# sahaRatul/sela

Hardware: AMD Instinct MI355X
Metric: Msamples/s encode+decode, 16-bit stereo 44.1kHz, 1/2/4/8 GPU; bit-exact vs CPU (higher is better)
Workload: dtype f64+int64

## Files before the change

### include/sela_hip_debug.h

```cpp
#ifndef SELA_HIP_DEBUG_H_
#define SELA_HIP_DEBUG_H_

#include <stddef.h>
#include <stdint.h>

#ifdef __cplusplus
extern "C" {
#endif

void sela_hip_debug_phase_buffer(uint64_t* d_cycles);
void sela_hip_debug_force_plain_fir(int enable);
void sela_hip_debug_mean_workers(int self_blocks);
void sela_hip_debug_encode_teams(int lanes);
int sela_hip_debug_encode_kernel(uint32_t n_frames, uint32_t channels);
void sela_hip_debug_encode_fused(int enable);
void sela_hip_debug_priorities(uint32_t team_quarters);
void sela_hip_debug_priorities_adaptive(void);
int sela_hip_debug_launches_alone(void);
void sela_hip_debug_keep_both_candidates(int on);
void sela_hip_debug_stage_wait(int naps);
int sela_hip_debug_reissued_feeds(void);
void sela_hip_debug_decode_recurrence(int form);
int sela_hip_debug_contexts_created(void);
void sela_hip_debug_coalesced(int kind, long long* batches, long long* retried);
size_t sela_hip_debug_verify_lds_bytes(uint32_t channels);
size_t sela_hip_debug_levels_lds_bytes(uint32_t channels);
size_t sela_hip_debug_digest_lds_bytes(uint32_t channels);
long long sela_hip_debug_verify_i32_fallback_frames(const void* d_workspace, uint32_t max_frames, uint32_t channels, uint32_t stride);
long long sela_hip_debug_verify_pcm_fallback_frames(const void* d_workspace, uint32_t max_frames, uint32_t channels, uint32_t stride);
long long sela_hip_debug_levels_i32_fallback_frames(const void* d_workspace, uint32_t max_frames, uint32_t channels, uint32_t stride);

void sela_hip_debug_encode_hashes(int on);
int sela_hip_debug_block_forms(const void* d_workspace, uint32_t n_frames, uint32_t channels, uint32_t* counts_out, uint8_t* forms_out);
void sela_hip_debug_encode_split(int mode);
int sela_hip_debug_launches_split(void);
void sela_hip_debug_standard_first(int mode);
int sela_hip_debug_standard_chunks(void);
long long sela_hip_debug_segment_subframes(void);
void sela_hip_debug_generic_wrap_taps(int on);
size_t sela_hip_debug_window_lds_bytes(uint32_t channels);
uint64_t sela_hip_debug_windows_staged_bytes(void);
enum {
    SELA_HIP_WORKSPACE_ENCODE = 0, SELA_HIP_WORKSPACE_DECODE, SELA_HIP_WORKSPACE_INDEX, SELA_HIP_WORKSPACE_DECODE_I32, SELA_HIP_WORKSPACE_DECODE_N,
    SELA_HIP_WORKSPACE_VERIFY, SELA_HIP_WORKSPACE_VERIFY_I32, SELA_HIP_WORKSPACE_ENCODE_I32, SELA_HIP_WORKSPACE_ENCODE_PAIRED, SELA_HIP_WORKSPACE_WINDOWS,
    SELA_HIP_WORKSPACE_WINDOWS_WHOLE, SELA_HIP_WORKSPACE_ENCODE_WHOLE, SELA_HIP_WORKSPACE_ENCODE_SPLIT, SELA_HIP_WORKSPACE_DECODE_WHOLE, SELA_HIP_WORKSPACE_WINDOWS_I32,
    SELA_HIP_WORKSPACE_WINDOWS_I32_WHOLE, SELA_HIP_WORKSPACE_ENCODE_WHOLE_PCM
};
int sela_hip_debug_workspace_pieces(int call, uint64_t a, uint32_t b, uint32_t c, uint64_t* offset_bytes_pairs, int capacity);
void sela_hip_debug_pcm_chunk_frames(uint32_t frames);

#ifdef __cplusplus
}
#endif
#endif
```

### sela_amd/capi.py

```python
from __future__ import annotations

import ctypes as C
import os

HERE = os.path.dirname(os.path.abspath(__file__))
LIB_PATH = os.path.join(HERE, "libsela_hip.so")

OK = 0
ERRORS = {-1: "ENODEV", -2: "EINVAL", -3: "ENOMEM", -4: "ECAPACITY", -5: "EFORMAT", -6: "ERANGE"}
SAMPLES_PER_FRAME = 2048

FLAG_Q_RANGE, FLAG_COEF_OVERFLOW, FLAG_RICE_RANGE, FLAG_RICE_OVERRUN, FLAG_WORDS_CAP, FLAG_BAD_FRAME, FLAG_INTERNAL, FLAG_SHORT_BLOCK = 1, 2, 4, 8, 16, 32, 64, 128
FLAG_STRIDE = 256

EXPORTS = [
    "sela_hip_init", "sela_hip_shutdown", "sela_hip_thread_release", "sela_hip_last_error", "sela_hip_device_count",
    "sela_hip_signals_per_frame", "sela_hip_encode_workspace_bytes", "sela_hip_decode_workspace_bytes",
    "sela_hip_encode_bound_bytes", "sela_hip_encode_device", "sela_hip_decode_device",
    "sela_hip_encode", "sela_hip_decode", "sela_hip_index_frames",
    "sela_hip_enable_kernel_timing", "sela_hip_kernel_times",
    "sela_hip_lpc_encode", "sela_hip_lpc_decode", "sela_hip_rice_encode", "sela_hip_rice_decode",
    "sela_hip_host_alloc", "sela_hip_host_free", "sela_hip_decode_max_channels",
    "sela_hip_encode_begin", "sela_hip_encode_feed", "sela_hip_encode_end",
    "sela_hip_decode_begin", "sela_hip_decode_feed", "sela_hip_decode_end",
# ... 6 lines not shown
    "sela_hip_verify_workspace_bytes", "sela_hip_verify_device", "sela_hip_verify_payload_device", "sela_hip_verify",
    "sela_hip_verify_i32_workspace_bytes", "sela_hip_verify_i32_device", "sela_hip_verify_payload_i32_device", "sela_hip_verify_i32",
    "sela_hip_encode_device_opt", "sela_hip_encode_n_device_opt", "sela_hip_encode_i32_device_opt", "sela_hip_encode_opt", "sela_hip_encode_i32_opt",
    "sela_hip_encode_ragged_i32_opt", "sela_hip_encode_begin_opt",
    "sela_hip_decode_windows_workspace_bytes", "sela_hip_decode_windows_device", "sela_hip_decode_windows",
    "sela_hip_decode_windows_whole_workspace_bytes", "sela_hip_decode_windows_whole_device", "sela_hip_decode_windows_whole",
    "sela_hip_decode_windows_i32_workspace_bytes", "sela_hip_decode_windows_i32_device", "sela_hip_decode_windows_i32",
    "sela_hip_decode_windows_i32_whole_workspace_bytes", "sela_hip_decode_windows_i32_whole_device", "sela_hip_decode_windows_i32_whole",
    "sela_hip_encode_whole_pcm_bound_bytes", "sela_hip_encode_whole_pcm_workspace_bytes", "sela_hip_encode_whole_pcm_device", "sela_hip_encode_whole_pcm",
    "sela_hip_paired_signals_per_frame", "sela_hip_encode_paired_workspace_bytes", "sela_hip_encode_paired_i32_device", "sela_hip_encode_paired_n_device",
    "sela_hip_encode_paired_i32", "sela_hip_encode_paired",
    "sela_hip_whole_frames", "sela_hip_whole_frame", "sela_hip_encode_whole_bound_bytes", "sela_hip_encode_whole_workspace_bytes",
    "sela_hip_encode_whole_device", "sela_hip_encode_whole",
    "sela_hip_decode_whole_workspace_bytes", "sela_hip_decode_whole_device", "sela_hip_decode_whole_payload_device", "sela_hip_decode_whole_status_error",
    "sela_hip_decode_whole",
    "sela_hip_pcm_unpack_device", "sela_hip_pcm_pack_device", "sela_hip_encode_pcm_workspace_bytes", "sela_hip_encode_pcm_bound_bytes",
    "sela_hip_encode_pcm_device", "sela_hip_decode_pcm_workspace_bytes", "sela_hip_decode_pcm_device", "sela_hip_decode_pcm_status_error",
    "sela_hip_encode_pcm", "sela_hip_decode_pcm",
    "sela_hip_verify_pcm_workspace_bytes", "sela_hip_verify_pcm_device", "sela_hip_verify_payload_pcm_device", "sela_hip_verify_pcm",
    "sela_hip_levels_workspace_bytes", "sela_hip_levels_device", "sela_hip_levels_payload_device", "sela_hip_levels",
    "sela_hip_levels_i32_workspace_bytes", "sela_hip_levels_i32_device", "sela_hip_levels_payload_i32_device", "sela_hip_levels_samples_i32_workspace_bytes",
    "sela_hip_levels_samples_i32_device", "sela_hip_levels_i32",
    "sela_hip_digest_workspace_bytes", "sela_hip_digest_device", "sela_hip_digest_payload_device", "sela_hip_digest", "sela_hip_crc32_combine",
    "sela_hip_crc32_workspace_bytes", "sela_hip_crc32_device",
]
WINDOW_I16_INTERLEAVED, WINDOW_F32_PLANAR = 0, 1
WINDOW_I32_PLANAR, WINDOW_PCM24_INTERLEAVED, WINDOW_PCM32_INTERLEAVED = 2, 3, 4
ENCODE_LOSSLESS = 1



DEBUG_EXPORTS = [
    "sela_hip_debug_phase_buffer", "sela_hip_debug_force_plain_fir", "sela_hip_debug_mean_workers", "sela_hip_debug_encode_teams", "sela_hip_debug_encode_kernel", "sela_hip_debug_encode_fused", "sela_hip_debug_priorities", "sela_hip_debug_priorities_adaptive", "sela_hip_debug_launches_alone", "sela_hip_debug_block_forms", "sela_hip_debug_encode_hashes", "sela_hip_debug_standard_first", "sela_hip_debug_standard_chunks", "sela_hip_debug_segment_subframes", "sela_hip_debug_generic_wrap_taps", "sela_hip_debug_encode_split", "sela_hip_debug_launches_split", "sela_hip_debug_keep_both_candidates", "sela_hip_debug_stage_wait",
    "sela_hip_debug_reissued_feeds", "sela_hip_debug_contexts_created", "sela_hip_debug_decode_recurrence", "sela_hip_debug_coalesced", "sela_hip_debug_verify_lds_bytes",
    "sela_hip_debug_verify_i32_fallback_frames", "sela_hip_debug_window_lds_bytes", "sela_hip_debug_windows_staged_bytes",
    "sela_hip_debug_workspace_pieces", "sela_hip_debug_pcm_chunk_frames", "sela_hip_debug_verify_pcm_fallback_frames",
    "sela_hip_debug_levels_lds_bytes", "sela_hip_debug_levels_i32_fallback_frames", "sela_hip_debug_digest_lds_bytes",
]
WORKSPACE_CALLS = ("encode", "decode", "index", "decode_i32", "decode_n", "verify", "verify_i32", "encode_i32", "encode_paired", "windows", "windows_whole",
                   "encode_whole", "encode_split", "decode_whole", "windows_i32", "windows_i32_whole", "encode_whole_pcm")


class Trace(C.Structure):
    _fields_ = [
        ("mean", C.c_double), ("ac", C.c_double * 101), ("k", C.c_double * 100), ("a", C.c_int64 * 101),
        ("q", C.c_int32 * 100), ("order", C.c_int32), ("coef_k", C.c_uint32), ("coef_words", C.c_uint32),
        ("res_k", C.c_uint32), ("res_words", C.c_uint32), ("flags", C.c_uint32),
    ]


class SelaHipError(RuntimeError):
    def __init__(self, code: int, message: str):
        super().__init__(f"libsela_hip: {ERRORS.get(code, code)}: {message}")
        self.code = code


_LIB = None


def lib() -> C.CDLL:
    global _LIB
    if _LIB is not None:
        return _LIB
    if not os.path.exists(LIB_PATH):
        raise ImportError(
            f"{LIB_PATH} is missing: build it with `python -c 'import __graft_entry__ as g; g.build()'` "
            "(hipcc --offload-arch=gfx950).  The SELA MI355X path has no CPU fallback.")
# ... 240 lines not shown
    L.sela_hip_debug_encode_fused.restype = None
    L.sela_hip_debug_priorities.argtypes = [C.c_uint32]
    L.sela_hip_debug_priorities.restype = None
    L.sela_hip_debug_priorities_adaptive.argtypes = []
    L.sela_hip_debug_priorities_adaptive.restype = None
    L.sela_hip_debug_launches_alone.argtypes = []
    L.sela_hip_debug_launches_alone.restype = C.c_int
    L.sela_hip_debug_encode_hashes.argtypes = [C.c_int]
    L.sela_hip_debug_encode_hashes.restype = None
    L.sela_hip_debug_standard_first.argtypes = [C.c_int]
    L.sela_hip_debug_standard_first.restype = None
    L.sela_hip_debug_standard_chunks.argtypes = []
    L.sela_hip_debug_standard_chunks.restype = C.c_int
    L.sela_hip_debug_segment_subframes.argtypes = []
    L.sela_hip_debug_segment_subframes.restype = C.c_longlong
    L.sela_hip_debug_generic_wrap_taps.argtypes = [C.c_int]
    L.sela_hip_debug_generic_wrap_taps.restype = None
    L.sela_hip_debug_encode_split.argtypes = [C.c_int]
    L.sela_hip_debug_encode_split.restype = None
    L.sela_hip_debug_launches_split.argtypes = []
    L.sela_hip_debug_launches_split.restype = C.c_int
    L.sela_hip_debug_block_forms.argtypes = [C.c_void_p, C.c_uint32, C.c_uint32, C.c_void_p, C.c_void_p]
    L.sela_hip_debug_block_forms.restype = C.c_int
    L.sela_hip_debug_keep_both_candidates.argtypes = [C.c_int]
    L.sela_hip_debug_keep_both_candidates.restype = None
    L.sela_hip_debug_encode_kernel.argtypes = [C.c_uint32, C.c_uint32]
    L.sela_hip_debug_encode_kernel.restype = C.c_int
    L.sela_hip_debug_stage_wait.argtypes = [C.c_int]
    L.sela_hip_debug_stage_wait.restype = None
    L.sela_hip_debug_reissued_feeds.argtypes = []
    L.sela_hip_debug_reissued_feeds.restype = C.c_int
    L.sela_hip_debug_decode_recurrence.argtypes = [C.c_int]
    L.sela_hip_debug_decode_recurrence.restype = None
    L.sela_hip_debug_contexts_created.argtypes = []
    L.sela_hip_debug_contexts_created.restype = C.c_int
    L.sela_hip_debug_coalesced.argtypes = [C.c_int, C.POINTER(C.c_longlong), C.POINTER(C.c_longlong)]
    L.sela_hip_debug_coalesced.restype = None
    L.sela_hip_debug_verify_lds_bytes.argtypes = [u32]
    L.sela_hip_debug_verify_lds_bytes.restype = sz
    L.sela_hip_debug_verify_i32_fallback_frames.argtypes = [vp, u32, u32, u32]
    L.sela_hip_debug_verify_pcm_fallback_frames.argtypes = [vp, u32, u32, u32]
    L.sela_hip_debug_verify_pcm_fallback_frames.restype = C.c_longlong
    L.sela_hip_debug_verify_i32_fallback_frames.restype = C.c_longlong
    L.sela_hip_debug_window_lds_bytes.argtypes = [u32]
    L.sela_hip_debug_window_lds_bytes.restype = sz
    L.sela_hip_debug_windows_staged_bytes.argtypes = []
    L.sela_hip_debug_windows_staged_bytes.restype = C.c_uint64
    L.sela_hip_debug_workspace_pieces.argtypes = [C.c_int, u64, u32, u32, u64p, C.c_int]
    L.sela_hip_debug_workspace_pieces.restype = C.c_int
    L.sela_hip_host_alloc.argtypes = [sz]
    L.sela_hip_host_alloc.restype = C.c_void_p
    L.sela_hip_host_free.argtypes = [C.c_void_p]
    L.sela_hip_host_free.restype = None
    L.sela_hip_decode_max_channels.argtypes = []
    L.sela_hip_decode_max_channels.restype = u32
    L.sela_hip_encode_begin.argtypes = [C.POINTER(C.c_void_p), u32, u32, vp, sz, vp]
    L.sela_hip_encode_feed.argtypes = [vp, vp, u32, C.POINTER(C.c_uint32), C.POINTER(C.c_uint64)]
    L.sela_hip_encode_end.argtypes = [vp, C.POINTER(C.c_uint32), C.POINTER(C.c_uint64)]
    L.sela_hip_decode_begin.argtypes = [C.POINTER(C.c_void_p), u32, u32, vp]
    L.sela_hip_decode_feed.argtypes = [vp, vp, vp, u32, C.POINTER(C.c_uint32)]
    L.sela_hip_decode_end.argtypes = [vp, C.POINTER(C.c_uint32)]
    for name in ("sela_hip_encode_begin", "sela_hip_encode_feed", "sela_hip_encode_end", "sela_hip_decode_begin",
                 "sela_hip_decode_feed", "sela_hip_decode_end"):
        getattr(L, name).restype = C.c_int
    _LIB = L
    return L
# ... 22 lines not shown
```

### sela_amd/csrc/sela_capi.hip

```cpp
#include <hip/hip_runtime.h>

#include <algorithm>
#include <atomic>

#include <chrono>
#include <condition_variable>
#include <deque>
#include <thread>
#include <cstdio>
#include <cstdlib>
#include <cstring>
#include <map>
#include <mutex>
#include <string>
#include <vector>

#include "sela_coalescer.h"
#include "sela_crc32.h"
#include "sela_decode_whole_plan.h"
#include "sela_host.h"
#include "sela_lease.h"
#include "sela_pcm.h"

namespace {
// ... 1147 lines not shown
    if (e == hipSuccess && blocks) {
        const size_t head = first ? (size_t)first * n_sig : blocks;
        if (!first)
            e = hipMemcpy(meta.data(), sela::encode_block_records(d_workspace, n_frames, channels), blocks * sizeof(sela::BlockMeta), hipMemcpyDeviceToHost);
        else {
            sela::Carve c(d_workspace);
            const SplitWs halves = carve_encode_split(c, first, n_frames - first, channels);
            e = hipMemcpy(meta.data(), sela::encode_block_records(halves.first, first, channels), head * sizeof(sela::BlockMeta), hipMemcpyDeviceToHost);
            if (e == hipSuccess)
                e = hipMemcpy(meta.data() + head, sela::encode_block_records(halves.second, n_frames - first, channels), (blocks - head) * sizeof(sela::BlockMeta),
                    hipMemcpyDeviceToHost);
        }
    }
    if (e != hipSuccess)
        return fail_hip(e, "block forms");
    for (size_t b = 0; b < blocks; b++) {
        const uint32_t form = (meta[b].flags & sela::kBlockFormPlain) ? 2 : ((meta[b].flags & sela::kBlockFormTwoPass) ? 1 : 0);
        counts_out[form]++;
        if (forms_out)
            forms_out[b] = (uint8_t)form;
    }
    return SELA_HIP_OK;
}
void sela_hip_debug_keep_both_candidates(int on) { sela::set_keep_both_candidates(on); }
void sela_hip_debug_encode_split(int mode) { g_encode_split.store(mode < 0 || mode > 999 ? 0 : mode, std::memory_order_relaxed); }
int sela_hip_debug_launches_split(void) { return g_launches_split.load(std::memory_order_relaxed); }
void sela_hip_debug_encode_hashes(int on) { sela::set_encode_hashes(on); }
int sela_hip_debug_encode_kernel(uint32_t n_frames, uint32_t channels) { return sela::encode_team_lanes(n_frames, channels, g_team_lanes); }

void sela_hip_debug_stage_wait(int naps) { g_stage_wait_naps = naps; }

int sela_hip_debug_reissued_feeds(void) { return g_reissued_feeds; }
void sela_hip_debug_decode_recurrence(int form) { g_recurrence_form = form < 0 ? -1 : (form != 0); }
int sela_hip_debug_contexts_created(void) { return g_contexts_created.load(std::memory_order_relaxed); }

void sela_hip_enable_kernel_timing(int enable) { g_timing.enabled = enable != 0; }

int sela_hip_kernel_times(float* ms_out, int capacity)
{
    const int n = g_timing.recorded < capacity ? g_timing.recorded : capacity;
    for (int i = 0; i < n; i++) {
        if (hipEventSynchronize(g_timing.ev[i + 1]) != hipSuccess || hipEventElapsedTime(&ms_out[i], g_timing.ev[i], g_timing.ev[i + 1]) != hipSuccess)
            return 0;
    }
    return n;
}

uint32_t sela_hip_signals_per_frame(uint32_t channels) { return channels == 2 ? 3u : channels; }

size_t sela_hip_encode_workspace_bytes(uint32_t n_frames, uint32_t channels)
{
    const size_t whole = sela::encode_workspace_bytes(n_frames, channels);
    return sela::encode_split_frames(n_frames, channels, 500) ? whole + sela::encode_workspace_bytes(0, channels) + 65536 : whole;
}

size_t sela_hip_decode_workspace_bytes(uint32_t n_frames, uint32_t channels) { return sela::decode_workspace_bytes(n_frames, channels); }

uint32_t sela_hip_decode_max_channels(void) { return sela::decode_max_channels(); }

size_t sela_hip_encode_bound_bytes(uint32_t n_frames, uint32_t channels)
{
    return (size_t)n_frames * sela_frame_bytes(channels, channels * (uint32_t)sela::kSlotWords);
}

namespace {
int encode_device_call(const int16_t* d_pcm, uint32_t n_frames, uint32_t channels, uint8_t* d_frames, size_t frames_cap,
// ... 2129 lines not shown
```

### sela_amd/csrc/sela_decode.hip

```cpp
#include <atomic>

#include "sela_host.h"

#include "sela_synth.h"

namespace sela {

#include "sela_decode_core.inc"

template <bool kProf>
__global__ __launch_bounds__(kDecMaxWaves * 64) __attribute__((amdgpu_waves_per_eu(7, 8))) void k_decode_frames(const uint8_t* __restrict__ frames,
    const uint64_t* __restrict__ frame_offsets, uint32_t n_frames, uint32_t channels, int16_t* __restrict__ pcm_out,
    uint32_t* __restrict__ status, int32_t* __restrict__ ws_residues, uint64_t* __restrict__ phase_cycles,
    uint8_t* __restrict__ frame_flags ,
    uint32_t vec_shift_from ,
    uint32_t synth_priorities ,
    const uint32_t* __restrict__ n_frames_found )
{
    long long stamp[10];
    for (int i = 0; i < 10; i++)
        stamp[i] = 0;
    uint32_t prof_sub = kNoSubframe;
    if (kProf)
        stamp[0] = clock64();
    extern __shared__ __attribute__((aligned(16))) unsigned char dyn[];
    const int n_waves = blockDim.x / 64;
    const int wave = __builtin_amdgcn_readfirstlane((int)(threadIdx.x / 64)), lane = threadIdx.x % 64;
    const DecFrameLds l = carve_frame_lds(dyn, channels, n_waves);

    const uint32_t f = blockIdx.x;
    if (f >= n_frames || (n_frames_found && f >= *n_frames_found))
        return;
    const bool vec_shift = f >= vec_shift_from;
    const uint8_t* const fb = frames + frame_offsets[f];
    const uint64_t fbytes = frame_offsets[f + 1] - frame_offsets[f];
    uint32_t flags = 0;
    SubHeader hd;
    bool ok;
    const bool fast = frame_prologue(l, fb, fbytes, channels, n_waves, wave, lane, hd, ok);
    if (kProf)
        stamp[1] = clock64();

    for (uint32_t c = wave; c < channels; c += n_waves) {
        if (c != (uint32_t)wave) {
            hd = walk_headers(fb, fbytes, c);
            ok = block_header_ok(hd, channels);
        }
        if (!ok) {
            flags |= SELA_HIP_FLAG_BAD_FRAME;
            continue;
        }
        if (kProf)
            prof_sub = c;
        decode_subframe<kProf>(fb, fbytes, hd, fast, l.sub + c, l.scratch0 + wave, ws_residues, (size_t)f * channels + c, vec_shift, synth_priorities, lane, flags, stamp);
        if (lane == 0)
            l.sub_info[hd.channel] = sub_info_word(hd.type, hd.parent, c);
    }
    __syncthreads();

    if (channels == 2) {
        const StereoPass sp = stereo_pass(l.sub, l.sub_info);
        uint4* out = reinterpret_cast<uint4*>(pcm_out + (size_t)f * kBlock * 2);
        for (uint32_t i4 = threadIdx.x; i4 < (uint32_t)kBlock / 4; i4 += blockDim.x)
            out[i4] = stereo_words(sp, i4);
    } else {
        for (uint32_t i = threadIdx.x; i < (uint32_t)kBlock; i += blockDim.x)
            for (uint32_t c = 0; c < channels; c++)
                pcm_out[((size_t)f * kBlock + i) * channels + c] = (int16_t)(uint16_t)channel_value16(l.sub, l.sub_info, c, i);
    }
    if (threadIdx.x == 0)
        flags |= layout_flags(l.sub_info, channels);
    flags = wave_or(flags);
    if (lane == 0 && flags) {
        if (frame_flags)
            frame_flags[(size_t)f * n_waves + wave] = (uint8_t)flags;
        else {
            atomicOr(&status[0], flags);
            if (wave == 0 && (flags & SELA_HIP_FLAG_BAD_FRAME))
                atomicAdd(&status[1], 1u);
        }
    }
    if (kProf && lane == 0 && prof_sub != kNoSubframe) {
        stamp[9] = clock64();
        for (int i = 0; i < 9; i++)
            phase_cycles[((size_t)f * channels + prof_sub) * 16 + i] = (uint64_t)(stamp[i + 1] - stamp[i]);
    }
}
// ... 36 lines not shown
    }
    asm volatile("s_waitcnt vmcnt(0)" ::: "memory");
    __syncthreads();
    __builtin_amdgcn_fence(__ATOMIC_ACQUIRE, "agent");
    for (uint32_t c = 0; c < channels; c++) {
        const uint32_t info = sub_info[c];
        if (info == kNoSubframe) {
            for (uint32_t i = threadIdx.x; i < (uint32_t)kBlock; i += blockDim.x)
                out_frame[(size_t)i * channels + c] = 0;
            if (threadIdx.x == 0)
                flags |= SELA_HIP_FLAG_BAD_FRAME;
        } else if (sub_info_type(info) == 1) {
            const uint32_t parent = sub_info_parent(info);
            const uint32_t pinfo = sub_info[parent];
            if (threadIdx.x == 0 && parent_refused(pinfo))
                flags |= SELA_HIP_FLAG_BAD_FRAME;
            for (uint32_t i = threadIdx.x; i < (uint32_t)kBlock; i += blockDim.x) {
                const uint32_t pv = pinfo == kNoSubframe ? 0u : (uint32_t)(uint16_t)out_frame[(size_t)i * channels + parent];
                const uint32_t dv = (uint32_t)(uint16_t)out_frame[(size_t)i * channels + c];
                out_frame[(size_t)i * channels + c] = (int16_t)(uint16_t)(pv - dv);
            }
        }
    }
    flags = wave_or(flags);
    if (lane == 0 && flags) {
        if (frame_flags)
            frame_flags[(size_t)f * kDecMaxWaves + wave] = (uint8_t)flags;
        else {
            atomicOr(&status[0], flags);
            if (wave == 0 && (flags & SELA_HIP_FLAG_BAD_FRAME))
                atomicAdd(&status[1], 1u);
        }
    }
}

int decode_waves(uint32_t channels)
{
    return channels < (uint32_t)kDecMaxWaves ? (int)channels : kDecMaxWaves;
}

size_t decode_lds_bytes(uint32_t channels) { return decode_lds_bytes_for(channels, decode_waves(channels)); }

uint32_t decode_max_channels() { return (uint32_t)kDecMaxChannels; }

int32_t* carve_decode(Carve& c, uint32_t n_frames, uint32_t channels) { return c.take<int32_t>((uint64_t)n_frames * channels * kBlock); }
size_t decode_workspace_bytes(uint32_t n_frames, uint32_t channels, Carve* at)
{
    return measured(at, [&](Carve& c) { carve_decode(c, n_frames, channels); });
}

struct DecodeResidency {
    std::atomic<uint32_t> frames[kResidencySlots][64][kDecMaxWaves + 1];
};
uint32_t resident_frames(const void* kernel, int n_waves, size_t lds, int slot)
{
    static DecodeResidency cache;
    int dev = 0;
    if (hipGetDevice(&dev) != hipSuccess || dev < 0 || dev >= 64 || slot < 0 || slot >= kResidencySlots || n_waves < 0 || n_waves > kDecMaxWaves)
        return 0;
    uint32_t have = cache.frames[slot][dev][n_waves].load(std::memory_order_relaxed);
    if (have == 0) {
        int per_cu = 0, cus = 0;
        if (hipOccupancyMaxActiveBlocksPerMultiprocessor(&per_cu, kernel, n_waves * 64, lds) != hipSuccess
            || hipDeviceGetAttribute(&cus, hipDeviceAttributeMultiprocessorCount, dev) != hipSuccess || per_cu <= 0 || cus <= 0)
            return 0;
        have = (uint32_t)per_cu * (uint32_t)cus;
// ... 94 lines not shown
    if (err != hipSuccess || n_frames == 0)
        return err;
    const int n_waves = decode_waves(channels);
    if (channels > (uint32_t)kDecMaxChannels)
        return hipErrorInvalidValue;
    Carve carve(d_workspace);
    int32_t* const ws = carve_decode(carve, n_frames, channels);
    if (channels > (uint32_t)kDecMaxWaves) {
        if (d_phase_cycles)
            return hipErrorInvalidValue;
        const size_t lds = (size_t)kDecMaxWaves * (sizeof(DecSubframeLds) + sizeof(DecWaveScratch)) + (size_t)channels * 4;
        if (ev)
            (void)hipEventRecord(ev[0], stream);
        const uint32_t from = recurrence_form >= 0 ? (recurrence_form ? 0u : n_frames)
                                                   : vec_shift_from_for(n_frames, kDecMaxWaves, resident_frames(reinterpret_cast<const void*>(k_decode_frames_wide), kDecMaxWaves, lds));
        hipLaunchKernelGGL(k_decode_frames_wide, dim3(n_frames), dim3(kDecMaxWaves * 64), lds, stream, d_frames, d_frame_offsets, n_frames, channels,
            d_pcm_out, d_status, ws, frame_flags, from, d_n_found);
        if (ev)
            (void)hipEventRecord(ev[1], stream);
        return hipGetLastError();
    }
    const size_t need = decode_lds_bytes(channels);
    const size_t lds = need;
    if (lds > 64 * 1024) {
        err = d_phase_cycles
            ? hipFuncSetAttribute(reinterpret_cast<const void*>(k_decode_frames<true>), hipFuncAttributeMaxDynamicSharedMemorySize, (int)lds)
            : hipFuncSetAttribute(reinterpret_cast<const void*>(k_decode_frames<false>), hipFuncAttributeMaxDynamicSharedMemorySize, (int)lds);
        if (err != hipSuccess)
            return err;
    }
    const uint32_t from = recurrence_form >= 0 ? (recurrence_form ? 0u : n_frames)
                                                : vec_shift_from_for(n_frames, n_waves, resident_frames(reinterpret_cast<const void*>(k_decode_frames<false>), n_waves, lds));
    const uint32_t synth_prio = synth_priorities;
    if (ev)
        (void)hipEventRecord(ev[0], stream);
    if (d_phase_cycles)
        hipLaunchKernelGGL(k_decode_frames<true>, dim3(n_frames), dim3(n_waves * 64), lds, stream, d_frames, d_frame_offsets, n_frames, channels,
            d_pcm_out, d_status, ws, d_phase_cycles, frame_flags, from, synth_prio, d_n_found);
    else
        hipLaunchKernelGGL(k_decode_frames<false>, dim3(n_frames), dim3(n_waves * 64), lds, stream, d_frames, d_frame_offsets, n_frames, channels,
            d_pcm_out, d_status, ws, d_phase_cycles, frame_flags, from, synth_prio, d_n_found);
    if (ev)
        (void)hipEventRecord(ev[1], stream);
    return hipGetLastError();
}

#include "sela_index.inc"

}
```

### sela_amd/csrc/sela_decode_core.inc

```

constexpr int kDecMaxWaves = 8;
constexpr int kDecMaxChannels = 255;
constexpr int kCoefLanes = 4;
constexpr int kResLanes = kWave - kCoefLanes;
constexpr int kStreamCap = 1072;
constexpr int kStreamMargin = 4;
constexpr uint32_t kEndOfStream = 0xFFFFFFFFu;

typedef uint32_t u32x4 __attribute__((ext_vector_type(4)));

struct SynthTables {
    union {
        int64_t a[104];
        uint64_t tab[192];
    };
};
struct DecWaveScratch {
    SynthTables t;
};
constexpr int kCoefValuesAt = 896;
static_assert(kCoefValuesAt + 104 * 4 <= (int)sizeof(SynthTables) && kCoefValuesAt >= 104 * 8, "the coefficient values lie behind a[] inside the table's space");
__device__ __forceinline__ int32_t* coef_values(DecWaveScratch* s)
{
    return reinterpret_cast<int32_t*>(reinterpret_cast<unsigned char*>(&s->t) + kCoefValuesAt);
// ... 335 lines not shown
__device__ inline SubHeader walk_to(const uint8_t* fb, uint64_t fbytes, HeaderCursor& cur, uint32_t c)
{
    SubHeader h;
    h.channel = h.type = h.parent = h.ck = h.cw = h.order = h.rk = h.rw = h.n = 0;
    h.ok = cur.ok;
    h.p = (uint32_t)cur.p;
    while (h.ok && cur.index <= c) {
        h.p = (uint32_t)cur.p;
        cur.p = sela_subframe_read_words(fb, fbytes, cur.p, &h);
        h.ok = cur.p != 0;
        cur.index++;
    }
    cur.ok = h.ok;
    return h;
}

__device__ inline SubHeader walk_headers(const uint8_t* fb, uint64_t fbytes, uint32_t c)
{
    HeaderCursor cur = frame_cursor(fb, fbytes);
    return walk_to(fb, fbytes, cur, c);
}

__device__ inline bool block_header_ok(const SubHeader& h, uint32_t channels)
{
    return h.ok && sela_subframe_decodable(&h) && h.n == (uint32_t)kBlock && h.channel < channels && h.type <= 1 && (h.type == 0 || h.parent < channels);
}

__device__ __forceinline__ bool predictor_table(uint32_t order, int32_t q_lo, int32_t q_hi, SynthTables* t, int lane, uint32_t& flags)
{
    step_up_from_q(order, q_lo, q_hi, t->a, lane, flags);
    return build_synth_table(t->a, t->tab, (int)order, lane);
}

template <bool kProf>
__device__ __forceinline__ void decode_subframe(const uint8_t* fb, uint64_t fbytes, const SubHeader& hd, bool fast, DecSubframeLds* sl, DecWaveScratch* scratch,
    int32_t* ws_residues, size_t ws_block, bool vec_shift, uint32_t synth_priorities , int lane, uint32_t& flags,
    long long* stamp )
{
    const uint32_t nw = hd.cw + 2 + hd.rw;
    const uint32_t* const gw = reinterpret_cast<const uint32_t*>(fb + hd.p + 4);
    const int32_t* ws_c = nullptr;
    ParseProfile pp;
    if (fast) {
        for (uint32_t w = lane; w < nw + kStreamMargin; w += kWave)
            sl->marks[w] = 0;
        wave_sync();
        if (kProf)
            stamp[2] = clock64();
        const StreamWords sw = { gw, nw };
        flags |= parse_subframe<kProf>(sw, sl->marks, sl->pos, reinterpret_cast<uint16_t*>(&scratch->t), coef_values(scratch), hd.cw, hd.rw, hd.ck, hd.rk,
            hd.order, lane, pp);
    } else {
        if (kProf)
            stamp[2] = clock64();
        int32_t* const wres = ws_residues + ws_block * kBlock;
        const uint32_t n_frame_words = (uint32_t)((fbytes - hd.p - 4) / 4);
        flags |= parse_stream_serial(gw, 24, 24 + 32 * hd.cw, n_frame_words, hd.ck, hd.order, coef_values(scratch), lane);
        flags |= parse_stream_serial(gw, 32 * (hd.cw + 2), 32 * (hd.cw + 2 + hd.rw), n_frame_words, hd.rk, (uint32_t)kBlock, wres, lane);
        asm volatile("s_waitcnt vmcnt(0)" ::: "memory");
        __builtin_amdgcn_fence(__ATOMIC_ACQUIRE, "agent");
        ws_c = wres;
        pp.t[0] = pp.t[1] = pp.t[2] = pp.t[3] = kProf ? clock64() : 0;
    }
    if (kProf)
        stamp[3] = pp.t[0], stamp[4] = pp.t[1], stamp[5] = pp.t[2], stamp[6] = pp.t[3];

    const uint32_t order = hd.order;
    const int32_t q_lo = (uint32_t)lane < order ? coef_values(scratch)[lane] : 0, q_hi = (uint32_t)lane + 64 < order ? coef_values(scratch)[lane + 64] : 0;
    wave_sync();
    const bool fits24 = predictor_table(order, q_lo, q_hi, &scratch->t, lane, flags);
    if (kProf)
        stamp[7] = clock64();
    if (synth_priorities)
        set_wave_priority((int)((synth_priorities >> (order <= 48 ? 0 : (order <= 60 ? 8 : 16))) & 0xFF));
    if (vec_shift)
        synthesize_by_order<true>(order, gw, nw, hd.rk, sl->pos, ws_c, scratch->t.tab, fits24, lane);
    else
        synthesize_by_order<false>(order, gw, nw, hd.rk, sl->pos, ws_c, scratch->t.tab, fits24, lane);
    if (synth_priorities)
        __builtin_amdgcn_s_setprio(0);
    if (kProf)
        stamp[8] = clock64();
}

constexpr uint32_t kNoSubframe = 0xFFFFFFFFu;
__device__ __forceinline__ uint32_t sub_info_word(uint32_t type, uint32_t parent, uint32_t position) { return type | (parent << 8) | (position << 16); }
__device__ __forceinline__ uint32_t sub_info_type(uint32_t info) { return info & 0xFF; }
__device__ __forceinline__ uint32_t sub_info_parent(uint32_t info) { return (info >> 8) & 0xFF; }
__device__ __forceinline__ uint32_t sub_info_position(uint32_t info) { return info >> 16; }

__host__ __device__ inline size_t decode_lds_bytes_for(uint32_t channels, int n_waves)
{
    return (size_t)channels * sizeof(DecSubframeLds) + (size_t)n_waves * sizeof(DecWaveScratch) + (size_t)channels * 4 + (size_t)n_waves * 4;
}
struct DecFrameLds {
    DecSubframeLds* sub;
    DecWaveScratch* scratch0;
    uint32_t* sub_info;
    uint32_t* too_big;
};
__device__ __forceinline__ DecFrameLds carve_frame_lds(unsigned char* dyn, uint32_t channels, int n_waves)
{
    DecFrameLds l;
    l.sub = reinterpret_cast<DecSubframeLds*>(dyn);
    l.scratch0 = reinterpret_cast<DecWaveScratch*>(dyn + (size_t)channels * sizeof(DecSubframeLds));
    l.sub_info = reinterpret_cast<uint32_t*>(dyn + (size_t)channels * sizeof(DecSubframeLds) + (size_t)n_waves * sizeof(DecWaveScratch));
    l.too_big = l.sub_info + channels;
    return l;
}

__device__ __forceinline__ bool frame_prologue(const DecFrameLds& l, const uint8_t* fb, uint64_t fbytes, uint32_t channels, int n_waves, int wave, int lane,
// ... 82 lines not shown
```

### sela_amd/csrc/sela_host.h

```cpp
#ifndef SELA_HOST_H_
#define SELA_HOST_H_

#include <string>

#include "sela_device.h"
#include "sela_generic.h"

namespace sela {

size_t encode_workspace_bytes(uint32_t n_frames, uint32_t channels, Carve* at = nullptr);
const BlockMeta* encode_block_records(const void* d_workspace, uint32_t n_frames, uint32_t channels);
int encode_team_lanes(uint32_t n_frames, uint32_t channels, int forced);
uint32_t encode_split_frames(uint32_t n_frames, uint32_t channels, int permille);
void set_keep_both_candidates(int on);
void set_encode_hashes(int on);
hipError_t launch_encode(const int16_t* d_pcm, uint32_t n_frames, uint32_t channels, uint8_t* d_frames, size_t frames_cap,
    uint64_t* d_frame_offsets, uint32_t* d_status, void* d_workspace, sela_hip_trace* d_trace, hipStream_t stream,
    hipEvent_t* ev, uint64_t* d_phase_cycles, const EncodeHostLink* link, int force_plain_fir, int self_blocks_override, int team_lanes,
    int32_t* d_trace_residues = nullptr, uint32_t priorities = 0, int phase = 0, const uint64_t* plan_base = nullptr, bool plan_accumulate = false,
    bool lossless = false);
hipError_t launch_stage_rice_encode(const int32_t* d_values, const uint64_t* d_value_offsets, uint32_t n_streams, uint32_t* d_k, uint32_t* d_word_counts,
    uint32_t* d_words, const uint64_t* d_word_offsets, uint32_t* d_status, hipStream_t stream);

int32_t* carve_decode(Carve& c, uint32_t n_frames, uint32_t channels);
size_t decode_workspace_bytes(uint32_t n_frames, uint32_t channels, Carve* at = nullptr);
uint32_t decode_max_channels();
hipError_t launch_decode(const uint8_t* d_frames, const uint64_t* d_frame_offsets, uint32_t n_frames, uint32_t channels,
    int16_t* d_pcm_out, uint32_t* d_status, void* d_workspace, hipStream_t stream, hipEvent_t* ev, uint64_t* d_phase_cycles,
    uint8_t* frame_flags, int recurrence_form, uint32_t synth_priorities = 0, const uint32_t* d_n_found = nullptr, bool zero_status = true);
hipError_t launch_stage_lpc_decode(const int32_t* d_order, const int32_t* d_q, const int32_t* d_residues, uint32_t n_blocks, int32_t* d_samples,
    int64_t* d_coefs, uint32_t* d_status, hipStream_t stream);
hipError_t launch_stage_rice_decode(const uint32_t* d_words, const uint64_t* d_word_offsets, const uint32_t* d_k, const uint64_t* d_value_offsets,
    uint32_t n_streams, int32_t* d_values, uint32_t* d_status, hipStream_t stream);
size_t index_workspace_bytes(uint64_t payload_bytes, Carve* at = nullptr);
hipError_t launch_index(const uint8_t* d_payload, uint64_t payload_bytes, uint32_t max_frames, uint32_t channels, uint64_t* d_frame_offsets,
    uint32_t* d_n_frames, void* d_workspace, hipStream_t stream);

uint32_t window_cover(uint32_t window_samples);
size_t window_workspace_bytes(uint32_t n_windows, uint32_t window_samples, uint32_t channels, Carve* at = nullptr);
hipError_t launch_window_frames(const uint8_t* d_frames, const uint64_t* d_frame_offsets, uint32_t n_frames_total, uint32_t channels, const sela_hip_window* d_windows,
    uint32_t n_windows, uint32_t window_samples, uint32_t format, void* d_out, uint32_t* d_window_flags, uint32_t* d_status, void* d_workspace, hipStream_t stream,
    int recurrence_form, uint32_t synth_priorities);
struct WindowWs {
    int32_t* residues;
    uint32_t* flag_words;
};
WindowWs carve_windows(Carve& c, uint32_t n_windows, uint32_t window_samples, uint32_t channels);

hipError_t launch_window_clear(uint32_t* d_status, uint32_t* d_window_flags , uint32_t n_windows, hipStream_t stream);

size_t window32_workspace_bytes(uint32_t n_windows, uint32_t window_samples, uint32_t channels, Carve* at = nullptr);
hipError_t launch_window32(const uint8_t* d_frames, const uint64_t* d_frame_offsets, uint32_t n_frames_total, uint32_t channels, const sela_hip_window* d_windows,
    uint32_t n_windows, uint32_t window_samples, uint32_t format, uint32_t sample_bits, void* d_out, uint32_t* d_window_flags, uint32_t* d_status, void* d_workspace,
    bool standard_path , hipStream_t stream);
struct TailSub;
struct Window32Ws {
    TailSub* subs;
    int32_t* dec;
    uint32_t* flag_words;
};
Window32Ws carve_window32(Carve& c, uint32_t n_windows, uint32_t window_samples, uint32_t channels);

// ... 119 lines not shown
```

### sela_amd/csrc/sela_synth.h

```cpp
#ifndef SELA_SYNTH_H_
#define SELA_SYNTH_H_

#include "sela_device.h"

namespace sela {

typedef const volatile __attribute__((address_space(3))) uint64_t* LdsTable;

__device__ __forceinline__ int32_t rice_value(uint32_t ones, uint32_t field, uint32_t k)
{
    const uint32_t rem = k ? (__brev(field) >> (32 - k)) : 0u;
    const uint32_t u = (ones << k) | rem;
    return (int32_t)((u >> 1) ^ (0u - (u & 1u)));
}

struct StreamWords {
    const uint32_t* words;
    uint32_t n_words;
};
__device__ __forceinline__ __amdgpu_buffer_rsrc_t stream_rsrc(const StreamWords& s)
{
    return __builtin_amdgcn_make_buffer_rsrc(
        reinterpret_cast<void*>(read_first_lane(reinterpret_cast<uint64_t>(s.words))), 0,
        4u * (uint32_t)__builtin_amdgcn_readfirstlane((int)s.n_words), 0x00020000);
// ... 179 lines not shown
    if constexpr (kOut32) {
#pragma unroll 1
        for (int pair = 0; pair < n_blocks; pair += R) {
            run_block(pair, zl[0], zh[0], zl[R - 1], zh[R - 1]);
            if (R == 2 && pair + 1 < n_blocks)
                run_block(pair + 1, zl[1], zh[1], zl[0], zh[0]);
        }
    } else {
#pragma unroll 1
        for (int blk = 0; blk < n_blocks; blk++) {
            run_block(blk, zl[0], zh[0], zl[R - 1], zh[R - 1]);
            if (R == 2) {
                const uint32_t tl = zl[0], th = zh[0];
                zl[0] = zl[1], zh[0] = zh[1];
                zl[1] = tl, zh[1] = th;
            }
        }
    }
    wave_sync();
}

template <bool kVecShift, bool kOut32 = false>
__device__ __forceinline__ void synthesize_by_order(uint32_t order, const uint32_t* words, uint32_t n_words, uint32_t k, uint16_t* pos_smp,
    const int32_t* ws, const uint64_t* tab, bool fold, int lane, SynthOut<kOut32> out32 = SynthOut<kOut32>())
{
    if (order <= 48)
        synthesize<1, 16, kVecShift, kOut32>(words, n_words, k, pos_smp, ws, tab, fold, lane, out32);
    else if (order <= 60)
        synthesize<1, 4, kVecShift, kOut32>(words, n_words, k, pos_smp, ws, tab, fold, lane, out32);
    else
        synthesize<2, 16, kVecShift, kOut32>(words, n_words, k, pos_smp, ws, tab, fold, lane, out32);
}

__device__ inline bool build_synth_table(const int64_t* a, uint64_t* tab, int order, int lane)
{
    uint64_t c[2];
    bool fits = true;
#pragma unroll
    for (int h = 0; h < 2; h++) {
        const int d = lane + 64 * h;
        const uint64_t nv = (uint64_t)(d >= 1 && d <= order ? a[d] : 0);
        const int32_t al = (int32_t)(uint32_t)nv;
        const int32_t ah = (int32_t)(uint32_t)((nv - (uint64_t)(int64_t)al) >> 32);
        fits &= ah >= -(1 << 23) && ah < (1 << 23);
        c[h] = ((uint64_t)(uint32_t)ah << 32) | (uint32_t)al;
    }
    wave_sync();
    if (order <= 60) {
        tab[lane] = c[0];
        tab[lane + 64] = c[0];
    } else {
        tab[lane] = c[0];
        tab[lane + 64] = c[1];
        tab[lane + 128] = c[0];
    }
    wave_sync();
    return !__any(!fits);
}

}

#endif
```

Baseline: 18360.

## Add fp64 FMA path for LPC synthesis in decode with integer fallback

```diff
diff --git a/include/sela_hip_debug.h b/include/sela_hip_debug.h
--- a/include/sela_hip_debug.h
+++ b/include/sela_hip_debug.h
@@ -21,6 +21,8 @@
 void sela_hip_debug_stage_wait(int naps);
 int sela_hip_debug_reissued_feeds(void);
 void sela_hip_debug_decode_recurrence(int form);
+void sela_hip_debug_decode_fp64(int mode);
+int sela_hip_debug_decode_fp64_counts(uint64_t* counts);
 int sela_hip_debug_contexts_created(void);
 void sela_hip_debug_coalesced(int kind, long long* batches, long long* retried);
 size_t sela_hip_debug_verify_lds_bytes(uint32_t channels);
diff --git a/sela_amd/capi.py b/sela_amd/capi.py
--- a/sela_amd/capi.py
+++ b/sela_amd/capi.py
@@ -62,7 +62,7 @@
 
 DEBUG_EXPORTS = [
     "sela_hip_debug_phase_buffer", "sela_hip_debug_force_plain_fir", "sela_hip_debug_mean_workers", "sela_hip_debug_encode_teams", "sela_hip_debug_encode_kernel", "sela_hip_debug_encode_fused", "sela_hip_debug_priorities", "sela_hip_debug_priorities_adaptive", "sela_hip_debug_launches_alone", "sela_hip_debug_block_forms", "sela_hip_debug_encode_hashes", "sela_hip_debug_standard_first", "sela_hip_debug_standard_chunks", "sela_hip_debug_segment_subframes", "sela_hip_debug_generic_wrap_taps", "sela_hip_debug_encode_split", "sela_hip_debug_launches_split", "sela_hip_debug_keep_both_candidates", "sela_hip_debug_stage_wait",
-    "sela_hip_debug_reissued_feeds", "sela_hip_debug_contexts_created", "sela_hip_debug_decode_recurrence", "sela_hip_debug_coalesced", "sela_hip_debug_verify_lds_bytes",
+    "sela_hip_debug_reissued_feeds", "sela_hip_debug_contexts_created", "sela_hip_debug_decode_recurrence", "sela_hip_debug_decode_fp64", "sela_hip_debug_decode_fp64_counts", "sela_hip_debug_coalesced", "sela_hip_debug_verify_lds_bytes",
     "sela_hip_debug_verify_i32_fallback_frames", "sela_hip_debug_window_lds_bytes", "sela_hip_debug_windows_staged_bytes",
     "sela_hip_debug_workspace_pieces", "sela_hip_debug_pcm_chunk_frames", "sela_hip_debug_verify_pcm_fallback_frames",
     "sela_hip_debug_levels_lds_bytes", "sela_hip_debug_levels_i32_fallback_frames", "sela_hip_debug_digest_lds_bytes",
@@ -369,6 +369,10 @@
     L.sela_hip_debug_reissued_feeds.restype = C.c_int
     L.sela_hip_debug_decode_recurrence.argtypes = [C.c_int]
     L.sela_hip_debug_decode_recurrence.restype = None
+    L.sela_hip_debug_decode_fp64.argtypes = [C.c_int]
+    L.sela_hip_debug_decode_fp64.restype = None
+    L.sela_hip_debug_decode_fp64_counts.argtypes = [C.POINTER(C.c_uint64)]
+    L.sela_hip_debug_decode_fp64_counts.restype = C.c_int
     L.sela_hip_debug_contexts_created.argtypes = []
     L.sela_hip_debug_contexts_created.restype = C.c_int
     L.sela_hip_debug_coalesced.argtypes = [C.c_int, C.POINTER(C.c_longlong), C.POINTER(C.c_longlong)]
diff --git a/sela_amd/csrc/sela_capi.hip b/sela_amd/csrc/sela_capi.hip
--- a/sela_amd/csrc/sela_capi.hip
+++ b/sela_amd/csrc/sela_capi.hip
@@ -1203,6 +1203,15 @@
 
 int sela_hip_debug_reissued_feeds(void) { return g_reissued_feeds; }
 void sela_hip_debug_decode_recurrence(int form) { g_recurrence_form = form < 0 ? -1 : (form != 0); }
+void sela_hip_debug_decode_fp64(int mode) { sela::set_decode_fp64(mode); }
+int sela_hip_debug_decode_fp64_counts(uint64_t* counts)
+{
+    unsigned long long c[4] = { 0, 0, 0, 0 };
+    const hipError_t e = counts ? sela::decode_fp64_counts(c) : hipErrorInvalidValue;
+    for (int i = 0; counts && i < 4; i++)
+        counts[i] = c[i];
+    return e == hipSuccess ? SELA_HIP_OK : SELA_HIP_ENODEV;
+}
 int sela_hip_debug_contexts_created(void) { return g_contexts_created.load(std::memory_order_relaxed); }
 
 void sela_hip_enable_kernel_timing(int enable) { g_timing.enabled = enable != 0; }
diff --git a/sela_amd/csrc/sela_decode.hip b/sela_amd/csrc/sela_decode.hip
--- a/sela_amd/csrc/sela_decode.hip
+++ b/sela_amd/csrc/sela_decode.hip
@@ -15,7 +15,8 @@
     uint8_t* __restrict__ frame_flags ,
     uint32_t vec_shift_from ,
     uint32_t synth_priorities ,
-    const uint32_t* __restrict__ n_frames_found )
+    const uint32_t* __restrict__ n_frames_found ,
+    unsigned long long* __restrict__ f64_counts )
 {
     long long stamp[10];
     for (int i = 0; i < 10; i++)
@@ -52,7 +53,8 @@
         }
         if (kProf)
             prof_sub = c;
-        decode_subframe<kProf>(fb, fbytes, hd, fast, l.sub + c, l.scratch0 + wave, ws_residues, (size_t)f * channels + c, vec_shift, synth_priorities, lane, flags, stamp);
+        decode_subframe<kProf, true>(fb, fbytes, hd, fast, l.sub + c, l.scratch0 + wave, ws_residues, (size_t)f * channels + c, vec_shift, synth_priorities, lane, flags, stamp,
+            f64_counts);
         if (lane == 0)
             l.sub_info[hd.channel] = sub_info_word(hd.type, hd.parent, c);
     }
@@ -155,6 +157,38 @@
                 atomicAdd(&status[1], 1u);
         }
     }
+}
+
+__device__ unsigned long long g_f64_counts[kF64CountSlots * kF64CountStride];
+static std::atomic<int> g_decode_fp64{ -1 };
+void set_decode_fp64(int mode) { g_decode_fp64.store(mode == 0 ? 0 : -1, std::memory_order_relaxed); }
+hipError_t decode_fp64_counts(unsigned long long* counts)
+{
+    unsigned long long all[kF64CountSlots * kF64CountStride];
+    hipError_t e = hipDeviceSynchronize();
+    if (e == hipSuccess)
+        e = hipMemcpyFromSymbol(all, HIP_SYMBOL(g_f64_counts), sizeof(all));
+    for (uint32_t i = 0; i < 4; i++) {
+        counts[i] = 0;
+        for (uint32_t slot = 0; e == hipSuccess && slot < kF64CountSlots; slot++)
+            counts[i] += all[slot * kF64CountStride + i];
+    }
+    return e;
+}
+static unsigned long long* f64_counts_for_launch()
+{
+    static std::atomic<unsigned long long*> known[64];
+    int dev = 0;
+    if (g_decode_fp64.load(std::memory_order_relaxed) == 0 || hipGetDevice(&dev) != hipSuccess || dev < 0 || dev >= 64)
+        return nullptr;
+    unsigned long long* have = known[dev].load(std::memory_order_relaxed);
+    if (!have) {
+        void* p = nullptr;
+        if (hipGetSymbolAddress(&p, HIP_SYMBOL(g_f64_counts)) != hipSuccess)
+            return nullptr;
+        known[dev].store(have = static_cast<unsigned long long*>(p), std::memory_order_relaxed);
+    }
+    return have;
 }
 
 int decode_waves(uint32_t channels)
@@ -315,14 +349,15 @@
     const uint32_t from = recurrence_form >= 0 ? (recurrence_form ? 0u : n_frames)
                                                 : vec_shift_from_for(n_frames, n_waves, resident_frames(reinterpret_cast<const void*>(k_decode_frames<false>), n_waves, lds));
     const uint32_t synth_prio = synth_priorities;
+    unsigned long long* const f64_counts = f64_counts_for_launch();
     if (ev)
         (void)hipEventRecord(ev[0], stream);
     if (d_phase_cycles)
         hipLaunchKernelGGL(k_decode_frames<true>, dim3(n_frames), dim3(n_waves * 64), lds, stream, d_frames, d_frame_offsets, n_frames, channels,
-            d_pcm_out, d_status, ws, d_phase_cycles, frame_flags, from, synth_prio, d_n_found);
+            d_pcm_out, d_status, ws, d_phase_cycles, frame_flags, from, synth_prio, d_n_found, f64_counts);
     else
         hipLaunchKernelGGL(k_decode_frames<false>, dim3(n_frames), dim3(n_waves * 64), lds, stream, d_frames, d_frame_offsets, n_frames, channels,
-            d_pcm_out, d_status, ws, d_phase_cycles, frame_flags, from, synth_prio, d_n_found);
+            d_pcm_out, d_status, ws, d_phase_cycles, frame_flags, from, synth_prio, d_n_found, f64_counts);
     if (ev)
         (void)hipEventRecord(ev[1], stream);
     return hipGetLastError();
diff --git a/sela_amd/csrc/sela_decode_core.inc b/sela_amd/csrc/sela_decode_core.inc
--- a/sela_amd/csrc/sela_decode_core.inc
+++ b/sela_amd/csrc/sela_decode_core.inc
@@ -391,10 +391,10 @@
     return build_synth_table(t->a, t->tab, (int)order, lane);
 }
 
-template <bool kProf>
+template <bool kProf, bool kF64 = false>
 __device__ __forceinline__ void decode_subframe(const uint8_t* fb, uint64_t fbytes, const SubHeader& hd, bool fast, DecSubframeLds* sl, DecWaveScratch* scratch,
     int32_t* ws_residues, size_t ws_block, bool vec_shift, uint32_t synth_priorities , int lane, uint32_t& flags,
-    long long* stamp )
+    long long* stamp , unsigned long long* f64_counts = nullptr )
 {
     const uint32_t nw = hd.cw + 2 + hd.rw;
     const uint32_t* const gw = reinterpret_cast<const uint32_t*>(fb + hd.p + 4);
@@ -432,10 +432,16 @@
         stamp[7] = clock64();
     if (synth_priorities)
         set_wave_priority((int)((synth_priorities >> (order <= 48 ? 0 : (order <= 60 ? 8 : 16))) & 0xFF));
+    bool in_f64 = false;
+    if constexpr (kF64)
+        in_f64 = !vec_shift && fast && f64_counts != nullptr;
     if (vec_shift)
         synthesize_by_order<true>(order, gw, nw, hd.rk, sl->pos, ws_c, scratch->t.tab, fits24, lane);
-    else
+    else if (!in_f64)
         synthesize_by_order<false>(order, gw, nw, hd.rk, sl->pos, ws_c, scratch->t.tab, fits24, lane);
+    if constexpr (kF64)
+        if (in_f64)
+            synthesize_f64_by_order(order, gw, nw, hd.rk, sl->pos, scratch->t.tab, fits24, lane, f64_counts);
     if (synth_priorities)
         __builtin_amdgcn_s_setprio(0);
     if (kProf)
diff --git a/sela_amd/csrc/sela_host.h b/sela_amd/csrc/sela_host.h
--- a/sela_amd/csrc/sela_host.h
+++ b/sela_amd/csrc/sela_host.h
@@ -28,6 +28,8 @@
 hipError_t launch_decode(const uint8_t* d_frames, const uint64_t* d_frame_offsets, uint32_t n_frames, uint32_t channels,
     int16_t* d_pcm_out, uint32_t* d_status, void* d_workspace, hipStream_t stream, hipEvent_t* ev, uint64_t* d_phase_cycles,
     uint8_t* frame_flags, int recurrence_form, uint32_t synth_priorities = 0, const uint32_t* d_n_found = nullptr, bool zero_status = true);
+void set_decode_fp64(int mode);
+hipError_t decode_fp64_counts(unsigned long long* counts);
 hipError_t launch_stage_lpc_decode(const int32_t* d_order, const int32_t* d_q, const int32_t* d_residues, uint32_t n_blocks, int32_t* d_samples,
     int64_t* d_coefs, uint32_t* d_status, hipStream_t stream);
 hipError_t launch_stage_rice_decode(const uint32_t* d_words, const uint64_t* d_word_offsets, const uint32_t* d_k, const uint64_t* d_value_offsets,
diff --git a/sela_amd/csrc/sela_synth.h b/sela_amd/csrc/sela_synth.h
--- a/sela_amd/csrc/sela_synth.h
+++ b/sela_amd/csrc/sela_synth.h
@@ -235,6 +235,206 @@
         synthesize<2, 16, kVecShift, kOut32>(words, n_words, k, pos_smp, ws, tab, fold, lane, out32);
 }
 
+template <int R, int G, int M>
+__device__ __forceinline__ void synth_steps_f64(double& zc, double& zo, uint32_t& kept, LdsTable tab_lane, uint32_t half_hi, uint32_t zero,
+    uint64_t (&pf_c)[kAhead], uint64_t (&pf_o)[kAhead])
+{
+    const uint32_t f_hi = (uint32_t)(__builtin_bit_cast(uint64_t, __builtin_floor(zc)) >> 32);
+    const double m_i = __builtin_bit_cast(double, (uint64_t)(uint32_t)__builtin_amdgcn_readlane((int)f_hi, M) << 32);
+    zc = __builtin_fma(__builtin_bit_cast(double, pf_c[M % kAhead]), m_i, zc);
+    if (R == 2)
+        zo = __builtin_fma(__builtin_bit_cast(double, pf_o[M % kAhead]), m_i, zo);
+    if constexpr (M + kAhead < 64) {
+        pf_c[M % kAhead] = tab_lane[64 * R - (M + kAhead)];
+        if (R == 2)
+            pf_o[M % kAhead] = tab_lane[64 - (M + kAhead)];
+    }
+    if constexpr ((M + 1) % G == 0) {
+        constexpr int first_lane = M + 1 - G;
+        constexpr int row_mask = 1 << (first_lane / 16);
+        constexpr int bank_mask = G == 16 ? 0xf : 1 << ((first_lane % 16) / 4);
+        const uint64_t z = __builtin_bit_cast(uint64_t, zc);
+        kept = (uint32_t)__builtin_amdgcn_update_dpp((int)kept, (int)f_hi, 0xE4 , row_mask, bank_mask, false);
+        const uint32_t hi = (uint32_t)__builtin_amdgcn_update_dpp((int)(uint32_t)(z >> 32), (int)half_hi, 0xE4, row_mask, bank_mask, false);
+        const uint32_t lo = (uint32_t)__builtin_amdgcn_update_dpp((int)(uint32_t)z, (int)zero, 0xE4, row_mask, bank_mask, false);
+        zc = __builtin_bit_cast(double, ((uint64_t)hi << 32) | lo);
+    }
+    __builtin_amdgcn_sched_barrier(0);
+    if constexpr (M < 63)
+        synth_steps_f64<R, G, M + 1>(zc, zo, kept, tab_lane, half_hi, zero, pf_c, pf_o);
+}
+
+template <int R, int G>
+__device__ __forceinline__ bool synth_block_f64(int32_t r_block, int32_t& s, double& zc, double& zo, LdsTable tab_lane, uint32_t half_hi, uint32_t zero, double sb)
+{
+    uint64_t pf_c[kAhead], pf_o[kAhead];
+#pragma unroll
+    for (int m = 0; m < kAhead; m++) {
+        pf_c[m] = tab_lane[64 * R - m];
+        pf_o[m] = R == 2 ? tab_lane[64 - m] : 0;
+    }
+    zc -= (double)r_block;
+    uint32_t kept = 0;
+    __builtin_amdgcn_sched_barrier(0);
+    synth_steps_f64<R, G, 0>(zc, zo, kept, tab_lane, half_hi, zero, pf_c, pf_o);
+    const double minus_s = __builtin_bit_cast(double, (uint64_t)kept << 32);
+    const bool within = __builtin_fabs(minus_s) <= sb;
+    s = within ? -(int32_t)minus_s : 0;
+    return !__any(!within);
+}
+
+__device__ __forceinline__ int64_t synth_coefficient(uint64_t packed)
+{
+    return (int64_t)((packed >> 32) << 32) + (int64_t)(int32_t)(uint32_t)packed;
+}
+__device__ __forceinline__ uint64_t synth_packed(int64_t a)
+{
+    const int32_t al = (int32_t)(uint32_t)(uint64_t)a;
+    const int32_t ah = (int32_t)(uint32_t)(((uint64_t)a - (uint64_t)(int64_t)al) >> 32);
+    return ((uint64_t)(uint32_t)ah << 32) | (uint32_t)al;
+}
+
+constexpr int32_t kF64ResidueBound = 1 << 16;
+constexpr double kF64Room = 0x1p53 - 0x1p34 - kF64ResidueBound * 0x1p35;
+constexpr uint32_t kF64Seen = 0, kF64Taken = 1, kF64Blocks = 2, kF64GivenUp = 3;
+constexpr uint32_t kF64CountSlots = 64, kF64CountStride = 8;
+
+template <int R, int G>
+__device__ __attribute__((noinline)) void synthesize_f64(const uint32_t* words, uint32_t n_words, uint32_t k, uint16_t* pos_smp, uint64_t* tab, bool fold,
+    int lane, unsigned long long* counts)
+{
+    static_assert(G == 4 || G == 16, "groups are DPP banks or rows");
+    const StreamWords sw = { words, n_words };
+    const __amdgpu_buffer_rsrc_t rs = stream_rsrc(sw);
+    k = (uint32_t)__builtin_amdgcn_readfirstlane((int)k);
+    const uint32_t kmask = k ? (0xFFFFFFFFu >> (32 - k)) : 0u;
+    const int64_t a0 = synth_coefficient(tab[lane]), a1 = R == 2 ? synth_coefficient(tab[lane + 64]) : 0;
+    const uint64_t m0 = (uint64_t)(a0 < 0 ? -a0 : a0), m1 = (uint64_t)(a1 < 0 ? -a1 : a1);
+    const bool small = !__any(m0 >= (1ull << 38) || m1 >= (1ull << 38));
+    const double sum_abs = (double)wave_sum_40(small ? m0 + m1 : 0);
+    double sb = __builtin_fmin(__builtin_floor(kF64Room / sum_abs), 2097151.0);
+    if (__builtin_fma(sb, sum_abs, -kF64Room) > 0.0)
+        sb -= 1.0;
+    sb = read_first_lane(sb);
+    bool f64 = small && sb >= 32768.0;
+    const bool taken = f64;
+    if (f64) {
+#pragma unroll
+        for (int h = 0; h < R + 1; h++)
+            tab[lane + 64 * h] = __builtin_bit_cast(uint64_t, (double)synth_coefficient(tab[lane + 64 * h]) * 0x1p-35);
+        wave_sync();
+    }
+    uint32_t zl[2], zh[2];
+#pragma unroll
+    for (int h = 0; h < 2; h++) {
+        zl[h] = 0;
+        zh[h] = f64 ? 0x3FE00000u : 4u;
+    }
+    uint32_t four = 4, zero = 0, half_hi = 0x3FE00000u;
+    asm volatile("" : "+v"(four), "+v"(zero), "+v"(half_hi));
+    const LdsTable tab_lane = (LdsTable)(tab + lane);
+    uint32_t p = 0, w0 = 0, w1 = 0, w2 = 0;
+    auto issue = [&](int blk) {
+        p = pos_smp[64 * blk + lane];
+        const uint32_t b = 4 * (p >> 5);
+        w0 = __builtin_amdgcn_raw_buffer_load_b32(rs, b, 0, 0);
+        w1 = __builtin_amdgcn_raw_buffer_load_b32(rs, b + 4, 0, 0);
+        w2 = __builtin_amdgcn_raw_buffer_load_b32(rs, b + 8, 0, 0);
+    };
+    auto land = [&]() -> int32_t {
+        uint32_t x0 = __builtin_amdgcn_alignbit(w1, w0, p & 31), x1 = __builtin_amdgcn_alignbit(w2, w1, p & 31), ones = 0;
+        while (__any(x0 == 0xFFFFFFFFu)) {
+            const bool more = x0 == 0xFFFFFFFFu;
+            ones += more ? 32u : 0u;
+            p += more ? 32u : 0u;
+            window64(rs, p, x0, x1);
+        }
+        const uint32_t t = (uint32_t)__builtin_ctz(~x0);
+        const uint32_t field = (uint32_t)(((((uint64_t)x1) << 32) | x0) >> (t + 1)) & kmask;
+        return rice_value(ones + t, field, k);
+    };
+    auto as_double = [](uint32_t lo, uint32_t hi) { return __builtin_bit_cast(double, ((uint64_t)hi << 32) | lo); };
+    constexpr int n_blocks = kBlock / 64;
+    uint32_t f64_blocks = 0;
+    issue(0);
+#pragma unroll 1
+    for (int blk = 0; blk < n_blocks; blk++) {
+        const int32_t r_block = land();
+        if (blk + 1 < n_blocks)
+            issue(blk + 1);
+        int32_t s;
+        bool done = false;
+        if (f64) {
+            if (!__any((uint32_t)(r_block + kF64ResidueBound) > 2u * (uint32_t)kF64ResidueBound)) {
+                double zc = as_double(zl[0], zh[0]), zo = as_double(zl[R - 1], zh[R - 1]);
+                done = synth_block_f64<R, G>(r_block, s, zc, zo, tab_lane, half_hi, zero, sb);
+                if (done) {
+                    const uint64_t c = __builtin_bit_cast(uint64_t, zc), o = __builtin_bit_cast(uint64_t, zo);
+                    zl[0] = (uint32_t)c, zh[0] = (uint32_t)(c >> 32);
+                    if (R == 2)
+                        zl[1] = (uint32_t)o, zh[1] = (uint32_t)(o >> 32);
+                    f64_blocks++;
+                }
+            }
+            if (!done) {
+                f64 = false;
+#pragma unroll
+                for (int h = 0; h < R; h++) {
+                    const int64_t n = (int64_t)(as_double(zl[h], zh[h]) * 0x1p35);
+                    zl[h] = (uint32_t)(uint64_t)n, zh[h] = (uint32_t)((uint64_t)n >> 32);
+                }
+#pragma unroll
+                for (int h = 0; h < R + 1; h++)
+                    tab[lane + 64 * h] = synth_packed((int64_t)(__builtin_bit_cast(double, tab[lane + 64 * h]) * 0x1p35));
+                wave_sync();
+            }
+        }
+        if (!done) {
+            fold = fold && !__any((uint32_t)(r_block + (1 << 23) - 1) >= (1u << 24) - 1u);
+            if (fold) {
+                const uint32_t s0 = zl[0], s1 = zh[0], s2 = zl[R - 1], s3 = zh[R - 1];
+                done = synth_block<R, true, G, false>(r_block, s, zl[0], zh[0], zl[R - 1], zh[R - 1], tab_lane, four, zero);
+                if (!done) {
+                    zl[0] = s0, zh[0] = s1;
+                    if (R == 2)
+                        zl[1] = s2, zh[1] = s3;
+                    fold = false;
+                }
+            }
+            if (!done)
+                synth_block<R, false, G, false>(r_block, s, zl[0], zh[0], zl[R - 1], zh[R - 1], tab_lane, four, zero);
+        }
+        reinterpret_cast<int16_t*>(pos_smp)[64 * blk + lane] = (int16_t)(uint16_t)(uint32_t)s;
+        if (R == 2) {
+            const uint32_t tl = zl[0], th = zh[0];
+            zl[0] = zl[1], zh[0] = zh[1];
+            zl[1] = tl, zh[1] = th;
+        }
+    }
+    if (lane == 0) {
+        unsigned long long* const c = counts + ((uint32_t)blockIdx.x % kF64CountSlots) * kF64CountStride;
+        __hip_atomic_fetch_add(c + kF64Seen, 1ull, __ATOMIC_RELAXED, __HIP_MEMORY_SCOPE_AGENT);
+        if (taken) {
+            __hip_atomic_fetch_add(c + kF64Taken, 1ull, __ATOMIC_RELAXED, __HIP_MEMORY_SCOPE_AGENT);
+            __hip_atomic_fetch_add(c + kF64Blocks, (unsigned long long)f64_blocks, __ATOMIC_RELAXED, __HIP_MEMORY_SCOPE_AGENT);
+            if (!f64)
+                __hip_atomic_fetch_add(c + kF64GivenUp, 1ull, __ATOMIC_RELAXED, __HIP_MEMORY_SCOPE_AGENT);
+        }
+    }
+    wave_sync();
+}
+
+__device__ __forceinline__ void synthesize_f64_by_order(uint32_t order, const uint32_t* words, uint32_t n_words, uint32_t k, uint16_t* pos_smp, uint64_t* tab,
+    bool fold, int lane, unsigned long long* counts)
+{
+    if (order <= 48)
+        synthesize_f64<1, 16>(words, n_words, k, pos_smp, tab, fold, lane, counts);
+    else if (order <= 60)
+        synthesize_f64<1, 4>(words, n_words, k, pos_smp, tab, fold, lane, counts);
+    else
+        synthesize_f64<2, 16>(words, n_words, k, pos_smp, tab, fold, lane, counts);
+}
+
 __device__ inline bool build_synth_table(const int64_t* a, uint64_t* tab, int order, int lane)
 {
     uint64_t c[2];
```

Measured after the change: 18430 (median of 6 runs). About the same (+0.4%).
